# knowles-group/iterative-solver

Hardware: AMD Instinct MI355X
Metric: subspace-update GB/s (gemm_inner+axpy) at N=1e8, 8 roots; 1/2/4/8 GPU (higher is better)
Workload: dtype f64

## Files before the change

iterative-solver_amd/csrc/context.hip:

```cpp
#include <immintrin.h>

#include <unistd.h>

#include <algorithm>
#include <atomic>
#include <chrono>
#include <condition_variable>
#include <cstdio>
#include <cstdlib>
#include <cstring>
#include <memory>
#include <mutex>
#include <thread>

#include "ssp_internal.h"

namespace {
thread_local std::string g_last_error;

size_t round_block(size_t bytes) {
  if (bytes < (size_t(1) << 20)) return (bytes + 255) & ~size_t(255);
  const size_t g = size_t(2) << 20;
  return (bytes + g - 1) / g * g;
}
// ... 287 lines not shown
}

int ledger_resolve(ssp_ctx* ctx) {
  SSP_TRY_HIP(hipStreamSynchronize(ctx->stream));
  for (auto& e : ctx->ledger) {
    for (auto& pr : e.pending) {
      float ms = 0;
      SSP_TRY_HIP(hipEventElapsedTime(&ms, pr.first, pr.second));
      e.ms += ms;
      ctx->event_pool.push_back(pr.first);
      ctx->event_pool.push_back(pr.second);
    }
    e.pending.clear();
  }
  return SSP_OK;
}
}

namespace {
thread_local LedgerScope* t_scope = nullptr;
}

LedgerScope::LedgerScope(ssp_ctx* ctx, const char* op, double bytes) : ctx_(ctx) {
  if (!ctx->ledger_on) return;
  slot_ = ledger_slot(ctx, op);
  ctx->ledger[slot_].calls += 1;
  ctx->ledger[slot_].bytes += bytes;
  last_bytes_ = bytes;
  start_ = take_event(ctx);
  if (!start_) return;
  if (ctx->ledger_dispatch) {
    stop_ = take_event(ctx);
    if (!stop_) {
      ctx->event_pool.push_back(start_);
      start_ = nullptr;
      return;
    }
    prev_ = t_scope;
    t_scope = this;
    return;
  }
  (void)hipEventRecord(start_, ctx->stream);
}

bool LedgerScope::dispatch_events(hipStream_t stream, hipEvent_t* start, hipEvent_t* stop) {
  LedgerScope* s = t_scope;
  if (!s || stream != s->ctx_->stream) return false;
  *start = s->launched_ ? nullptr : s->start_;
  *stop = s->stop_;
  s->launched_ = true;
  return true;
}

void LedgerScope::detail(const std::string& tag) {
  if (slot_ < 0 || !ctx_->ledger_detail) return;
  const std::string name = ctx_->ledger[slot_].name + " [" + tag + "]";
  auto& from = ctx_->ledger[slot_];
  from.calls -= 1;
  const double b = last_bytes_;
  from.bytes -= b;
  const int to = ledger_slot(ctx_, name.c_str());
  ctx_->ledger[to].calls += 1;
  ctx_->ledger[to].bytes += b;
  slot_ = to;
}

LedgerScope::~LedgerScope() {
  if (slot_ < 0 || !start_) return;
  if (stop_) {
    t_scope = prev_;
    if (!launched_) {
      ctx_->event_pool.push_back(start_);
      ctx_->event_pool.push_back(stop_);
      return;
    }
    ctx_->ledger[slot_].pending.emplace_back(start_, stop_);
  } else {
    hipEvent_t end = take_event(ctx_);
    if (!end) return;
    (void)hipEventRecord(end, ctx_->stream);
    ctx_->ledger[slot_].pending.emplace_back(start_, end);
  }
  if (ctx_->ledger[slot_].pending.size() > 4096) (void)ledger_resolve(ctx_);
}

}

extern "C" {

int ssp_ledger_enable(ssp_ctx* ctx, int enable) {
  SSP_CHECK_CTX(ctx);
  ctx->ledger_on = enable != 0;
  return SSP_OK;
}

int ssp_ledger_reset(ssp_ctx* ctx) {
  SSP_CHECK_CTX(ctx);
  SSP_TRY(ssp::ledger_resolve(ctx));
  ctx->ledger.clear();
  return SSP_OK;
}

int ssp_ledger_reserve(ssp_ctx* ctx, int n) {
  SSP_CHECK_CTX(ctx);
  SSP_TRY(ssp::use_device(ctx));
  while (int(ctx->event_pool.size()) < n) {
    hipEvent_t e = nullptr;
    SSP_TRY_HIP(hipEventCreate(&e));
    ctx->event_pool.push_back(e);
  }
  return SSP_OK;
}

int ssp_ledger_count(ssp_ctx* ctx) {
  if (!ctx) return -1;
// ... 4 lines not shown
int ssp_ledger_entry(ssp_ctx* ctx, int i, const char** name, long long* calls, double* kernel_ms, double* bytes) {
  SSP_CHECK_CTX(ctx);
  SSP_TRY(ssp::ledger_resolve(ctx));
  if (i < 0 || size_t(i) >= ctx->ledger.size()) return ssp::set_error(SSP_ERR_ARG, "ssp_ledger_entry: bad index");
  const auto& e = ctx->ledger[i];
  if (name) *name = e.name.c_str();
  if (calls) *calls = e.calls;
  if (kernel_ms) *kernel_ms = e.ms;
  if (bytes) *bytes = e.bytes;
  return SSP_OK;
}

const char* ssp_last_error(void) { return g_last_error.c_str(); }

const char* ssp_version(void) { return "subspace_hip 0.1 (gfx950, fp64)"; }

int ssp_device_count(void) {
  int n = 0;
  if (hipGetDeviceCount(&n) != hipSuccess) return 0;
  return n;
}

int ssp_ctx_create(int device, ssp_ctx** out) {
  if (!out) return ssp::set_error(SSP_ERR_ARG, "ssp_ctx_create: null out");
  *out = nullptr;
  int ndev = 0;
  SSP_TRY_HIP(hipGetDeviceCount(&ndev));
  if (device < 0 || device >= ndev)
    return ssp::set_error(SSP_ERR_ARG, "ssp_ctx_create: device " + std::to_string(device) + " not present");
  SSP_TRY_HIP(hipSetDevice(device));
  auto* ctx = new ssp_ctx();
  ctx->device = device;
  hipDeviceProp_t prop;
  if (hipGetDeviceProperties(&prop, device) == hipSuccess && prop.multiProcessorCount > 0)
    ctx->num_cus = prop.multiProcessorCount;
  if (const char* rs = std::getenv("SSP_ROW_SHAPE")) ctx->row_stride = std::string(rs) == "stride";
  if (const char* pc = std::getenv("SSP_PUBLISH")) ctx->publish_copy = std::string(pc) == "copy";
  if (const char* ex = std::getenv("SSP_EXACT_MAX")) ctx->exact_max = size_t(std::strtoull(ex, nullptr, 10));
  if (const char* ip = std::getenv("SSP_INNER_PER_CU")) ctx->inner_per_cu = std::max(1, std::atoi(ip));
  if (const char* op = std::getenv("SSP_OUTER_WG_PER_CU")) ctx->outer_per_cu = std::max(1, std::atoi(op));
  if (const char* fp = std::getenv("SSP_FUSED_PER_CU")) ctx->fused_per_cu = std::max(1, std::atoi(fp));
  if (const char* tw = std::getenv("SSP_TRANSFORM_WIDE")) ctx->transform_wide = std::atoi(tw) != 0;
  if (const char* sm = std::getenv("SSP_SELECT_MERGE")) ctx->select_rank = std::string(sm) != "tree";
  if (const char* lt = std::getenv("SSP_LEDGER_TIMING")) ctx->ledger_dispatch = std::string(lt) == "dispatch";
  ctx->ledger_detail = std::getenv("SSP_LEDGER_DETAIL") != nullptr;
  if (const char* ss = std::getenv("SSP_SYNTH_SHAPE")) {
    ctx->synth_stride = std::string(ss) == "stride";
    ctx->synth_window = std::string(ss) == "window";
  }
  if (const char* sm = std::getenv("SSP_SYNTH_MERGE")) ctx->synth_merge = std::atoi(sm) != 0;
  if (const char* df = std::getenv("SSP_DEFER_FILL")) ctx->defer_fill = std::atoi(df) != 0;
  if (const char* dout = std::getenv("SSP_DEFER_OUTER")) ctx->outer.defer = std::atoi(dout) != 0;
  if (const char* on = std::getenv("SSP_OUTER_NORMS")) ctx->outer.norms_on = std::atoi(on) != 0;
  if (const char* ct = std::getenv("SSP_COMM_TIMEOUT_S")) {
    const double v = std::atof(ct);
    if (v > 0) ctx->comm_timeout_s = v;
  }
  if (hipStreamCreateWithFlags(&ctx->stream, hipStreamNonBlocking) != hipSuccess) {
    delete ctx;
    return ssp::set_error(SSP_ERR_HIP, "hipStreamCreate failed");
  }
  int s = ssp::ensure_partial(ctx, size_t(1) << 20);
  if (s == SSP_OK) s = ssp::ensure_result(ctx, size_t(1) << 16);
  if (s == SSP_OK) {
    const size_t bytes = sizeof(unsigned) * ssp::kFoldLine * (ssp::kFoldShards + 1);
    if (hipMalloc(reinterpret_cast<void**>(&ctx->fold_counter), bytes) != hipSuccess ||
        hipMemsetAsync(ctx->fold_counter, 0, bytes, ctx->stream) != hipSuccess)
      s = ssp::set_error(SSP_ERR_NOMEM, "allocation of the reduction counter failed");
  }
  if (s != SSP_OK) {
    ssp_ctx_destroy(ctx);
    return s;
  }
  *out = ctx;
  return SSP_OK;
}

int ssp_ctx_destroy(ssp_ctx* ctx) {
  if (!ctx) return SSP_OK;
  (void)hipSetDevice(ctx->device);
  ctx->pending_fills.clear();
  ctx->outer.pending.discard();
  (void)ssp::p2p_detach(ctx);
  if (ctx->stream) (void)hipStreamSynchronize(ctx->stream);
  if (ctx->comm) ncclCommDestroy(ctx->comm);
  if (ctx->dev_err_host) (void)hipHostFree(ctx->dev_err_host);
  for (auto& e : ctx->ledger)
    for (auto& pr : e.pending) {
      (void)hipEventDestroy(pr.first);
      (void)hipEventDestroy(pr.second);
    }
  for (auto ev : ctx->event_pool) (void)hipEventDestroy(ev);
  for (auto& b : ctx->free_blocks) (void)hipFree(b.second);
  for (auto& b : ctx->live_blocks) (void)hipFree(b.first);
  if (ctx->partial) (void)hipFree(ctx->partial);
  if (ctx->outer.norms_dev) (void)hipFree(ctx->outer.norms_dev);
  if (ctx->result_dev) (void)hipFree(ctx->result_dev);
  if (ctx->result_host) (void)hipHostFree(ctx->result_host);
  if (ctx->pub_flag) (void)hipHostFree(ctx->pub_flag);
  if (ctx->fold_counter) (void)hipFree(ctx->fold_counter);
  if (ctx->async_dev) (void)hipFree(ctx->async_dev);
  if (ctx->async_host) (void)hipHostFree(ctx->async_host);
  if (ctx->async_flag) (void)hipHostFree(ctx->async_flag);
  if (ctx->synth_mask) (void)hipFree(ctx->synth_mask);
  if (ctx->ring_dev) (void)hipFree(ctx->ring_dev);
  if (ctx->ring_host) (void)hipHostFree(ctx->ring_host);
  for (auto& r : ctx->retired_rings) {
    if (r.first) (void)hipFree(r.first);
    if (r.second) (void)hipHostFree(r.second);
  }
  if (ctx->stream) (void)hipStreamDestroy(ctx->stream);
  delete ctx;
  return SSP_OK;
}

void* ssp_ctx_stream(ssp_ctx* ctx) {
  if (!ctx) return nullptr;
  (void)ssp::enter(ctx);
  return reinterpret_cast<void*>(ctx->stream);
}

int ssp_synchronize(ssp_ctx* ctx) {
  SSP_CHECK_CTX(ctx);
  return ssp::sync_stream(ctx, "synchronize");
}

int ssp_alloc(ssp_ctx* ctx, size_t n, double** out) {
  SSP_CHECK_CTX(ctx);
  if (!out) return ssp::set_error(SSP_ERR_ARG, "ssp_alloc: null out");
  const size_t bytes = round_block(std::max<size_t>(n, 1) * sizeof(double));
  auto it = ctx->free_blocks.find(bytes);
  void* p = nullptr;
  if (it != ctx->free_blocks.end()) {
    p = it->second;
    ctx->free_blocks.erase(it);
// ... 222 lines not shown
```

iterative-solver_amd/csrc/kernels_outer.hip:

```cpp
#include <algorithm>
#include <string>
#include <vector>

#include "ssp_internal.h"

namespace {

using ssp::kBlock;
using ssp::ld2, ssp::sc1, ssp::sc2;

struct OuterArgs {
  const double* x[ssp::kOuterSrc];
  double* y[ssp::kOuterDst];
  int k;
  int m;
  int set;
  int epi_mask;
  size_t n;
  const double* alpha_dev;
  const double* scale_dev;
  double alpha[ssp::kOuterAlpha];
  double epi[ssp::kOuterDst];
  double* partial;
  ssp::FoldTail tail;
// ... 166 lines not shown
          *reinterpret_cast<double2*>(a.y[j] + 2 * p) = v;
          double s = nacc[j * U * kBlock];
          s = fma(v.x, v.x, s);
          s = fma(v.y, v.y, s);
          nacc[j * U * kBlock] = s;
        }
      }
      if ((a.n & 1) && threadIdx.x == 0) {
        const size_t e = a.n - 1;
        for (int j = 0; j < a.m; ++j) {
          double v = 0.0;
          for (int i = 0; i < a.k; ++i) v = fma(alpha(i * a.m + j), a.x[i][e], v);
          if constexpr (EPI) {
            if ((a.epi_mask >> j) & 1) v = fma(a.epi[j], a.x[a.k + j][e], v);
          }
          a.y[j][e] = v;
          nacc[j * U * kBlock] = fma(v, v, nacc[j * U * kBlock]);
        }
      }
    }
    __shared__ double red[kBlock / 64][M];
#pragma unroll
    for (int j = 0; j < M; ++j)
      if (j < a.m) {
        const double s0 = nacc[(j * U + 0) * kBlock], s1 = nacc[(j * U + 1) * kBlock];
        const double s2 = nacc[(j * U + 2) * kBlock], s3 = nacc[(j * U + 3) * kBlock];
        double v = (s0 + s1) + (s2 + s3);
#pragma unroll
        for (int off = 32; off > 0; off >>= 1) v += __shfl_down(v, off, 64);
        if (lane == 0) red[threadIdx.x >> 6][j] = v;
      }
    __syncthreads();
    if (int(threadIdx.x) < a.m) {
      double s = 0;
#pragma unroll
      for (int w = 0; w < kBlock / 64; ++w) s += red[w][threadIdx.x];
      ssp::store_partial(a.partial + size_t(blockIdx.x) * a.m + threadIdx.x, s);
    }
    ssp::fold_tail<M>(a.partial, a.tail);
    return;
  }
  if ((a.n & 1) && blockIdx.x == 0 && threadIdx.x < a.m) {
    const size_t e = a.n - 1;
    const int j = threadIdx.x;
    double v = SET ? 0.0 : sc1<SC>(a.y[j][e], scale(a.k + j));
    for (int i = 0; i < a.k; ++i) v = fma(alpha(i * a.m + j), sc1<SC>(a.x[i][e], scale(i)), v);
    if constexpr (EPI) {
      if ((a.epi_mask >> j) & 1) v = fma(a.epi[j], a.x[a.k + j][e], v);
    }
    a.y[j][e] = v;
  }
}

constexpr int kOuterNormDst = 8;
unsigned outer_norm_grid(const ssp_ctx* ctx, size_t n) { return ssp::win_grid(ctx, n, ssp::kDotU, 8); }

int outer_inst(int m) { return m <= 1 ? 1 : m <= 2 ? 2 : m <= 4 ? 4 : m <= 8 ? 8 : 16; }

template <int M, bool DEV, bool SET, bool SC, bool EPI, bool NRM>
void launch_outer_inst(ssp_ctx* ctx, unsigned grid, const OuterArgs& a) {
  SSP_LAUNCH((k_gemm_outer<M, DEV, SET, SC, EPI, NRM>), dim3(grid), dim3(kBlock), 0, ctx->stream, a);
}

template <bool DEV, bool SET, bool SC, bool EPI = false, bool NRM = false>
void launch_outer_m(ssp_ctx* ctx, unsigned grid, const OuterArgs& a) {
  switch (outer_inst(a.m)) {
    case 1: return launch_outer_inst<1, DEV, SET, SC, EPI, NRM>(ctx, grid, a);
    case 2: return launch_outer_inst<2, DEV, SET, SC, EPI, NRM>(ctx, grid, a);
    case 4: return launch_outer_inst<4, DEV, SET, SC, EPI, NRM>(ctx, grid, a);
    case 8: return launch_outer_inst<8, DEV, SET, SC, EPI, NRM>(ctx, grid, a);
    default:
      if constexpr (!NRM) launch_outer_inst<16, DEV, SET, SC, EPI, NRM>(ctx, grid, a);
  }
}

template <bool SET, bool SC, bool EPI = false, bool NRM = false>
void launch_outer_dev(ssp_ctx* ctx, unsigned grid, const OuterArgs& a) {
  a.alpha_dev ? launch_outer_m<true, SET, SC, EPI, NRM>(ctx, grid, a)
              : launch_outer_m<false, SET, SC, EPI, NRM>(ctx, grid, a);
}

int launch_outer(ssp_ctx* ctx, const OuterArgs& a) {
  const unsigned grid = a.partial ? outer_norm_grid(ctx, a.n)
                                  : ssp::stream_grid(ctx, a.n / 2 + 1, kOuterWin, unsigned(ctx->outer_per_cu));
  if (a.partial) {
    if (!a.set || a.scale_dev || a.m > kOuterNormDst || (a.epi_mask && a.k + a.m > ssp::kOuterSrc))
      return ssp::set_error(SSP_ERR_ARG, "gemm_outer: norms on a launch that cannot carry them");
    a.epi_mask ? launch_outer_dev<true, false, true, true>(ctx, grid, a)
               : launch_outer_dev<true, false, false, true>(ctx, grid, a);
  } else if (a.epi_mask) {
    if (!a.set || a.scale_dev || a.k + a.m > ssp::kOuterSrc)
      return ssp::set_error(SSP_ERR_ARG, "gemm_outer: epilogue terms on a launch that cannot carry them");
    launch_outer_dev<true, false, true>(ctx, grid, a);
  } else if (a.scale_dev) {
    a.set ? launch_outer_dev<true, true>(ctx, grid, a) : launch_outer_dev<false, true>(ctx, grid, a);
  } else {
    a.set ? launch_outer_dev<true, false>(ctx, grid, a) : launch_outer_dev<false, false>(ctx, grid, a);
  }
  SSP_TRY_HIP(hipGetLastError());
  return SSP_OK;
}

int outer_args(ssp_ctx* ctx, const double* alphas, const double* const* xx, const double* xs, int k,
               double* const* yy, const double* ys, int m, size_t n, bool set0, int i0, int j0, OuterArgs* out,
               std::string* tag) {
  OuterArgs& a = *out;
  a = OuterArgs{};
// ... 2 lines not shown
  a.set = (set0 && i0 == 0) ? 1 : 0;
  a.n = n;
  for (int i = 0; i < a.k; ++i) a.x[i] = xx[i0 + i];
  for (int j = 0; j < a.m; ++j) a.y[j] = yy[j0 + j];
  if (xs || ys) {
    std::vector<double> scl(size_t(a.k + a.m), 1.0);
    for (int i = 0; i < a.k; ++i) scl[size_t(i)] = xs ? xs[i0 + i] : 1.0;
    for (int j = 0; j < a.m; ++j) scl[size_t(a.k + j)] = (ys && i0 == 0 && !set0) ? ys[j0 + j] : 1.0;
    if (ssp::any_scaled(scl.data(), int(scl.size()))) {
      void* ps;
      SSP_TRY(ssp::upload_small(ctx, scl.data(), scl.size() * sizeof(double), &ps));
      a.scale_dev = static_cast<const double*>(ps);
    }
  }
  const bool dev = a.k * a.m > ssp::kOuterAlpha;
  std::vector<double> block(dev ? size_t(a.k) * a.m : 0);
  double* dst = dev ? block.data() : a.alpha;
  for (int i = 0; i < a.k; ++i)
    for (int j = 0; j < a.m; ++j) dst[i * a.m + j] = alphas[size_t(i0 + i) * m + j0 + j];
  if (dev) {
    void* p;
    SSP_TRY(ssp::upload_small(ctx, block.data(), block.size() * sizeof(double), &p));
    a.alpha_dev = static_cast<const double*>(p);
  }
  SSP_TRY(ssp::flush_uploads(ctx));
  *tag = ssp::shape_tag(dev ? "dev" : "arg", outer_inst(a.m), a.set, a.k, a.m, a.scale_dev != nullptr);
  return SSP_OK;
}

int launch_record(ssp_ctx* ctx, const ssp::PendingOuter::Record& r, const ssp::FoldTail* norms = nullptr) {
  const int e = r.terms();
  ssp::LedgerScope ls(ctx, r.set ? "gemm_outer_set" : "gemm_outer", 8.0 * r.n * (r.k + r.m + e));
  OuterArgs a;
  std::string tag;
  SSP_TRY(outer_args(ctx, r.alpha, r.x, nullptr, r.k, r.y, nullptr, r.m, r.n, true, 0, 0, &a, &tag));
  if (e > 0) {
    a.epi_mask = int(r.mask);
    for (int j = 0; j < r.m; ++j) {
      const bool on = (r.mask >> j) & 1u;
      a.x[r.k + j] = on ? r.ex[j] : nullptr;
      a.epi[j] = on ? r.ea[j] : 0.0;
    }
    tag += " epi" + std::to_string(e);
  }
  if (norms) {
    a.partial = ctx->partial;
    a.tail = *norms;
    tag += " nrm";
  }
  ls.detail(tag);
  return launch_outer(ctx, a);
}

int launch_outer_norms(ssp_ctx* ctx, const double* y, size_t n) {
  ssp::DeferredOuter& d = ctx->outer;
  if (!d.norms_on || !d.pending.pending()) return SSP_OK;
  const ssp::PendingOuter::Record& r = d.pending.record();
  const int m = r.m;
  if (m > kOuterNormDst || n != r.n || std::find(r.y, r.y + m, y) == r.y + m) return SSP_OK;
  d.norms.forget();
  const bool ranks = ssp::comm_attached(ctx);
  ssp::FoldTail tail{};
  int status = ssp::ensure_partial(ctx, size_t(outer_norm_grid(ctx, r.n)) * m);
  if (status == SSP_OK) status = ssp::fold_begin(ctx, m, &tail);
  if (status == SSP_OK && ranks) {
    if (!d.norms_dev && hipMalloc(reinterpret_cast<void**>(&d.norms_dev), ssp::kOuterDst * sizeof(double)) != hipSuccess)
      status = ssp::set_error(SSP_ERR_NOMEM, "hipMalloc of the norm staging failed");
    tail.out = d.norms_dev;
  }
  if (status != SSP_OK) {
    const int plain = ssp::flush_outer(ctx);
    return plain != SSP_OK ? plain : status;
  }
  d.norms.keep(r.y, m, r.n);
  d.pending.flush([&](const ssp::PendingOuter::Record& rec) { status = launch_record(ctx, rec, &tail); });
  if (status == SSP_OK && !ranks) {
    double v[ssp::kOuterDst];
    status = ssp::fold_finish(ctx, tail, v);
    if (status == SSP_OK) d.norms.set_values(v);
  }
  if (status != SSP_OK) d.norms.forget();
  return status;
}

}

namespace ssp {

int flush_outer(ssp_ctx* ctx) {
  DeferredOuter& d = ctx->outer;
  d.norms.forget();
  if (!d.pending.pending()) return SSP_OK;
  int status = SSP_OK;
  d.pending.flush([&](const PendingOuter::Record& r) { status = launch_record(ctx, r); });
  return status;
}

int outer_take_axpy(ssp_ctx* ctx, double alpha, const double* x, double xs, double* y, double ys, size_t n,
                    bool* attached) {
  DeferredOuter& d = ctx->outer;
  *attached = false;
  d.norms.forget();
  if (!d.pending.pending()) return SSP_OK;
  const bool valid = n > 0 && x && y && aligned16(x) && aligned16(y);
  if (valid && xs == 1.0 && ys == 1.0 && d.pending.attach(alpha, x, y, n)) {
    *attached = true;
    return flush_fills_over(ctx, x, n);
  }
  return flush_outer(ctx);
}

int outer_serve_dot(ssp_ctx* ctx, const double* x, double xs, const double* y, double ys, size_t n, double* out,
                    bool* served) {
  DeferredOuter& d = ctx->outer;
  *served = false;
  if (!out || x != y || xs != 1.0 || ys != 1.0) return SSP_OK;
  SSP_TRY(launch_outer_norms(ctx, y, n));
  const int j = d.norms.find(y, n);
  if (j < 0) return SSP_OK;
  *served = true;
  if (!comm_attached(ctx)) {
    *out = d.norms.value(j);
    return SSP_OK;
  }
  SSP_TRY(comm_check(ctx));
  SSP_TRY(ensure_result(ctx, 1));
  SSP_TRY_HIP(hipMemcpyAsync(ctx->result_dev, d.norms_dev + j, sizeof(double), hipMemcpyDeviceToDevice, ctx->stream));
  return reduce_fetch(ctx, out, 1);
}

}

namespace {
int gemm_outer_impl(ssp_ctx* ctx, const double* alphas, const double* const* xx, const double* xs, int k,
                    double* const* yy, const double* ys, int m, size_t n, bool set) {
  SSP_CHECK_CTX_KEEP_FILLS(ctx);
  if (m < 0 || k < 0) return ssp::set_error(SSP_ERR_ARG, "ssp_gemm_outer: negative dimension");
  if (set && k == 0) {
    for (int j = 0; j < m; ++j) SSP_TRY(ssp_fill(ctx, 0.0, yy[j], n));
    return SSP_OK;
  }
  if (m == 0 || n == 0) return SSP_OK;
  if (k == 0) {
    for (int j = 0; j < m; ++j)
      if (!set && ys && ys[j] != 1.0) SSP_TRY(ssp_scal(ctx, ys[j], yy[j], n));
    return SSP_OK;
  }
  if (!alphas) return ssp::set_error(SSP_ERR_ARG, "ssp_gemm_outer: null alphas");
  SSP_TRY(ssp::check_ptrs(xx, k, n, "ssp_gemm_outer"));
  SSP_TRY(ssp::check_ptrs(yy, m, n, "ssp_gemm_outer"));
  for (int j = 0; j < m; ++j)
    for (int i = 0; i < k; ++i)
      if (yy[j] == xx[i]) return ssp::set_error(SSP_ERR_ARG, "ssp_gemm_outer: a destination aliases a source");
  bool consume = false;
  if (!ctx->pending_fills.empty()) {
    for (int i = 0; i < k; ++i) SSP_TRY(ssp::flush_fills_over(ctx, xx[i], n));
    if (set) {
      for (int j = 0; j < m; ++j) SSP_TRY(ssp::overwrite_fills(ctx, yy[j], n));
    } else {
      consume = !ssp::any_scaled(ys, m) && !ssp::exact_mode(ctx, n);
      for (int j = 0; consume && j < m; ++j) {
        consume = ctx->pending_fills.find_exact(yy[j], n) >= 0;
        for (int i = 0; consume && i < j; ++i) consume = yy[i] != yy[j];
      }
      for (int j = 0; j < m; ++j) {
        if (consume) ctx->pending_fills.erase(ctx->pending_fills.find_exact(yy[j], n));
        else SSP_TRY(ssp::flush_fills_over(ctx, yy[j], n));
      }
    }
  }
  const bool set0 = set || consume;
  if (ctx->outer.defer && set0 && !ssp::any_scaled(xs, k) && !ssp::exact_mode(ctx, n) &&
      ctx->outer.pending.record(alphas, xx, k, yy, m, n, set))
    return SSP_OK;
  ssp::LedgerScope ls(ctx, set ? "gemm_outer_set" : "gemm_outer", 8.0 * n * (k + (set0 ? 1.0 : 2.0) * m));
  if (ssp::exact_mode(ctx, n)) return ssp::exact_outer(ctx, alphas, xx, xs, k, yy, ys, m, n, set);
  for (int j0 = 0; j0 < m; j0 += ssp::kOuterDst)
    for (int i0 = 0; i0 < k; i0 += ssp::kOuterSrc) {
      OuterArgs a;
      std::string tag;
      SSP_TRY(outer_args(ctx, alphas, xx, xs, k, yy, ys, m, n, set0, i0, j0, &a, &tag));
      if (j0 == 0 && i0 == 0) ls.detail(tag);
      SSP_TRY(launch_outer(ctx, a));
    }
  return SSP_OK;
}
}

extern "C" {

int ssp_gemm_outer(ssp_ctx* ctx, const double* alphas, const double* const* xx, int k, double* const* yy, int m,
                   size_t n) {
  return gemm_outer_impl(ctx, alphas, xx, nullptr, k, yy, nullptr, m, n, false);
}

int ssp_gemm_outer_set(ssp_ctx* ctx, const double* alphas, const double* const* xx, int k, double* const* yy, int m,
                       size_t n) {
  return gemm_outer_impl(ctx, alphas, xx, nullptr, k, yy, nullptr, m, n, true);
}

int ssp_gemm_outer_scaled(ssp_ctx* ctx, const double* alphas, const double* const* xx, const double* xs, int k,
                          double* const* yy, const double* ys, int m, size_t n) {
  return gemm_outer_impl(ctx, alphas, xx, xs, k, yy, ys, m, n, false);
}

int ssp_gemm_outer_set_scaled(ssp_ctx* ctx, const double* alphas, const double* const* xx, const double* xs, int k,
                              double* const* yy, int m, size_t n) {
  return gemm_outer_impl(ctx, alphas, xx, xs, k, yy, nullptr, m, n, true);
}

}
```

iterative-solver_amd/csrc/kernels_stream.hip:

```cpp
#include <algorithm>
#include <cmath>

#include "ssp_internal.h"

namespace {

using ssp::kBlock;
using ssp::ld2, ssp::sc1, ssp::sc2, ssp::st2;
using ssp::kWinMin;
using ssp::kWinU;
using ssp::kDotU;

__device__ __forceinline__ double block_sum(double v) {
  __shared__ double wsum[kBlock / 64];
#pragma unroll
  for (int off = 32; off > 0; off >>= 1) v += __shfl_down(v, off, 64);
  const int lane = threadIdx.x & 63, wave = threadIdx.x >> 6;
  if (lane == 0) wsum[wave] = v;
  __syncthreads();
  double s = 0;
  if (threadIdx.x == 0) {
#pragma unroll
    for (int w = 0; w < kBlock / 64; ++w) s += wsum[w];
  }
// ... 270 lines not shown
    SSP_TRY_HIP(hipGetLastError());
    return SSP_OK;
  }
  SSP_LAUNCH(k_reduce_partials, dim3(rows * cols), dim3(kBlock), 0, ctx->stream, partial, nblocks, rows, cols,
                     out, ldo, row0, col0);
  SSP_TRY_HIP(hipGetLastError());
  return SSP_OK;
}
int fill_now(ssp_ctx* ctx, double alpha, double* x, size_t n) {
  SSP_TRY(ssp::check_vec(x, n, "ssp_fill"));
  if (n == 0) return SSP_OK;
  LedgerScope ls(ctx, "fill", 8.0 * n);
  SSP_LAUNCH(k_fill, dim3(stream_grid(ctx, n / 2 + 1, 1, 64)), dim3(kBlock), 0, ctx->stream, x, n, alpha);
  SSP_TRY_HIP(hipGetLastError());
  return SSP_OK;
}

namespace {
struct FillFlusher {
  ssp_ctx* ctx;
  int status = SSP_OK;
  void operator()(double* p, size_t n) {
    const int s = fill_now(ctx, 0.0, p, n);
    if (status == SSP_OK) status = s;
  }
};
}

int flush_fills(ssp_ctx* ctx) {
  if (ctx->pending_fills.empty()) return SSP_OK;
  FillFlusher f{ctx};
  ctx->pending_fills.drain(f);
  return f.status;
}

int flush_fills_over(ssp_ctx* ctx, const void* p, size_t n) {
  if (ctx->pending_fills.empty()) return SSP_OK;
  FillFlusher f{ctx};
  ctx->pending_fills.flush_overlap(p, n, f);
  return f.status;
}

int overwrite_fills(ssp_ctx* ctx, const void* p, size_t n) {
  if (ctx->pending_fills.empty()) return SSP_OK;
  FillFlusher f{ctx};
  ctx->pending_fills.overwrite(p, n, f);
  return f.status;
}
}

extern "C" {

int ssp_fill(ssp_ctx* ctx, double alpha, double* x, size_t n) {
  SSP_CHECK_CTX_KEEP_FILLS(ctx);
  if (ctx->defer_fill && n > 0 && alpha == 0.0 && !std::signbit(alpha) && !ssp::exact_mode(ctx, n)) {
    SSP_TRY(ssp::check_vec(x, n, "ssp_fill"));
    ssp::FillFlusher f{ctx};
    ctx->pending_fills.insert(x, n, f);
    return f.status;
  }
  SSP_TRY(ssp::overwrite_fills(ctx, x, n));
  return ssp::fill_now(ctx, alpha, x, n);
}

int ssp_scal(ssp_ctx* ctx, double alpha, double* x, size_t n) {
  SSP_CHECK_CTX(ctx);
  SSP_TRY(ssp::check_vec(x, n, "ssp_scal"));
  if (n == 0) return SSP_OK;
  ssp::LedgerScope ls(ctx, "scal", 16.0 * n);
  if (n >= kWinMin)
    SSP_LAUNCH(k_scal_win, dim3(ssp::win_grid(ctx, n, kWinU, 16)), dim3(kBlock), 0, ctx->stream, x, n, alpha);
  else
    SSP_LAUNCH(k_scal, dim3(ssp::stream_grid(ctx, n / 2 + 1, 4, 64)), dim3(kBlock), 0, ctx->stream, x, n, alpha);
  SSP_TRY_HIP(hipGetLastError());
  return SSP_OK;
}

}

namespace {
int copy_impl(ssp_ctx* ctx, double alpha, double* x, const double* y, size_t n, bool scaled, const char* what) {
  SSP_CHECK_CTX_KEEP_FILLS(ctx);
  SSP_TRY(ssp::check_vec(x, n, what));
  SSP_TRY(ssp::check_vec(y, n, what));
  if (n == 0 || (x == y && !scaled)) return SSP_OK;
  if (x == y) return ssp_scal(ctx, alpha, x, n);
  SSP_TRY(ssp::flush_fills_over(ctx, y, n));
  SSP_TRY(ssp::overwrite_fills(ctx, x, n));
  ssp::LedgerScope ls(ctx, scaled ? "scal_copy" : "copy", 16.0 * n);
  if (n >= kWinMin) {
    const dim3 g(ssp::win_grid(ctx, n, kWinU, 16));
    if (scaled) SSP_LAUNCH(k_copy_win<true>, g, dim3(kBlock), 0, ctx->stream, x, y, n, alpha);
    else SSP_LAUNCH(k_copy_win<false>, g, dim3(kBlock), 0, ctx->stream, x, y, n, alpha);
  } else {
    const dim3 g(ssp::stream_grid(ctx, n / 2 + 1, 4, 64));
    if (scaled) SSP_LAUNCH(k_copy<true>, g, dim3(kBlock), 0, ctx->stream, x, y, n, alpha);
    else SSP_LAUNCH(k_copy<false>, g, dim3(kBlock), 0, ctx->stream, x, y, n, alpha);
  }
  SSP_TRY_HIP(hipGetLastError());
  return SSP_OK;
}

int axpy_impl(ssp_ctx* ctx, double alpha, const double* x, double xs, double* y, double ys, size_t n,
              const char* what) {
  SSP_CHECK_CTX_KEEP_ALL(ctx);
  bool attached = false;
  SSP_TRY(ssp::outer_take_axpy(ctx, alpha, x, xs, y, ys, n, &attached));
  if (attached) return SSP_OK;
// ... 112 lines not shown
```

iterative-solver_amd/csrc/pending_outer.h:

```cpp
#pragma once
#include <cstddef>
#include <cstdint>

namespace ssp {

class PendingOuter {
 public:
  static constexpr int kSrc = 64;
  static constexpr int kDst = 16;

  struct Record {
    double alpha[kSrc * kDst];
    const double* x[kSrc];
    double* y[kDst];
    int k = 0;
    int m = 0;
    size_t n = 0;
    bool set = false;
    double ea[kDst];
    const double* ex[kDst];
    unsigned mask = 0;

    int terms() const {
      int e = 0;
      for (int j = 0; j < m; ++j) e += (mask >> j) & 1u;
      return e;
    }
  };

  bool pending() const { return pending_; }
  const Record& record() const { return r_; }

  static bool one_launch(int k, int m) { return k >= 1 && m >= 1 && k <= kSrc && m <= kDst; }
  static bool epilogue_fits(int k, int m) { return k + m <= kSrc; }

  bool record(const double* alphas, const double* const* xx, int k, double* const* yy, int m, size_t n, bool set) {
    if (pending_ || n == 0 || !one_launch(k, m)) return false;
    for (int j = 0; j < m; ++j)
      for (int i = 0; i < j; ++i)
        if (overlap(yy[i], yy[j], n)) return false;
    for (int i = 0; i < k * m; ++i) r_.alpha[i] = alphas[i];
    for (int i = 0; i < k; ++i) r_.x[i] = xx[i];
    for (int j = 0; j < m; ++j) r_.y[j] = yy[j];
    r_.k = k;
    r_.m = m;
    r_.n = n;
    r_.set = set;
    r_.mask = 0;
    pending_ = true;
    return true;
  }

  bool attach(double alpha, const double* x, const double* y, size_t n) {
    if (!pending_ || n != r_.n || !epilogue_fits(r_.k, r_.m)) return false;
    int j = 0;
    while (j < r_.m && r_.y[j] != y) ++j;
    if (j == r_.m || ((r_.mask >> j) & 1u)) return false;
    for (int d = 0; d < r_.m; ++d)
      if (overlap(x, r_.y[d], n)) return false;
    r_.ea[j] = alpha;
    r_.ex[j] = x;
    r_.mask |= 1u << j;
    return true;
  }

  template <typename F>
  void flush(F&& launch) {
    if (!pending_) return;
    pending_ = false;
    launch(static_cast<const Record&>(r_));
  }

  void discard() { pending_ = false; }

 private:
  static bool overlap(const void* a, const void* b, size_t n) {
    const uintptr_t p = reinterpret_cast<uintptr_t>(a), q = reinterpret_cast<uintptr_t>(b);
    const size_t bytes = n * sizeof(double);
    return p < q + bytes && q < p + bytes;
  }

  Record r_;
  bool pending_ = false;
};

}
```

iterative-solver_amd/csrc/ssp_internal.h:

```cpp
#pragma once
#include <hip/hip_ext.h>
#include <hip/hip_runtime.h>
#include <rccl/rccl.h>

#include <cstddef>
#include <cstdint>
#include <map>
#include <string>
#include <unordered_map>
#include <vector>

#include "pending_fill.h"
#include "pending_outer.h"
#include "outer_norms.h"
#include "subspace_hip.h"

struct ssp_ledger_entry_t {
  std::string name;
  long long calls = 0;
  double ms = 0;
  double bytes = 0;
  std::vector<std::pair<hipEvent_t, hipEvent_t>> pending;
};

namespace ssp {
struct P2PComm;

struct DeferredOuter {
  bool defer = true;
  PendingOuter pending;
  bool norms_on = true;
  OuterNorms norms;
  double* norms_dev = nullptr;
};
}

struct ssp_ctx {
  int device = 0;
  bool ledger_on = false;
  std::vector<ssp_ledger_entry_t> ledger;
  std::vector<hipEvent_t> event_pool;
  int num_cus = 256;
  int inner_per_cu = 4;
  int outer_per_cu = 8;
  int fused_per_cu = 8;
  bool select_rank = true;
  bool transform_wide = true;
  bool synth_stride = false;
  bool ledger_dispatch = false;
  bool ledger_detail = false;
  bool synth_window = false;
  bool synth_merge = true;
  bool row_stride = false;
  bool publish_copy = false;
  bool defer_fill = true;
  ssp::PendingFills pending_fills;
  ssp::DeferredOuter outer;
  hipStream_t stream = nullptr;

  std::multimap<size_t, void*> free_blocks;
  std::unordered_map<void*, size_t> live_blocks;
  size_t bytes_in_use = 0;
  size_t bytes_cached = 0;

  double* partial = nullptr;
  size_t partial_cap = 0;
  double* result_dev = nullptr;
  double* result_host = nullptr;
  size_t result_cap = 0;
  unsigned long long* pub_flag = nullptr;
  unsigned long long pub_seq = 0;
  unsigned* fold_counter = nullptr;
  double* async_dev = nullptr;
  double* async_host = nullptr;
  unsigned long long* async_flag = nullptr;
  unsigned long long async_seq = 0;
  bool async_pending = false;
  bool async_launched = false;
  size_t async_n = 0;
  std::vector<double> async_sync;

  char* ring_host = nullptr;
  char* ring_dev = nullptr;
  size_t ring_cap = 0;
  size_t ring_head = 0;
  size_t ring_pending = 0;
  std::vector<std::pair<char*, char*>> retired_rings;

  unsigned short* synth_mask = nullptr;
  size_t synth_mask_n = 0, synth_mask_offset = 0;
  unsigned long long synth_mask_seed = 0;
  int synth_mask_rank = 0;

  ncclComm_t comm = nullptr;
  ssp_host_allreduce_fn host_allreduce = nullptr;
  ssp_host_allgather_fn host_allgather = nullptr;
  void* host_user = nullptr;
  ssp::P2PComm* p2p = nullptr;
  int nranks = 1;
  int rank = 0;
  double comm_timeout_s = 300.0;
  size_t exact_max = 2048;
  bool comm_failed = false;
  std::string comm_fail_msg;
  int* dev_err_host = nullptr;
};

namespace ssp {

constexpr int kBlock = 256;
constexpr int kInnerRows = 16;
constexpr int kInnerCols = 64;
constexpr int kOuterSrc = 64;
constexpr int kOuterDst = 16;
constexpr int kOuterAlpha = 384;
constexpr int kPrecVec = 16;
constexpr int kSelectTile = 2048;
constexpr int kWinU = 8;
constexpr size_t kWinMin = size_t(1) << 24;
constexpr int kDotU = 4;

int set_error(int code, const std::string& msg);
int hip_error(hipError_t e, const char* what);
int use_device(ssp_ctx* ctx);
int fill_now(ssp_ctx* ctx, double alpha, double* x, size_t n);
int flush_fills(ssp_ctx* ctx);
int flush_fills_over(ssp_ctx* ctx, const void* p, size_t n);
int overwrite_fills(ssp_ctx* ctx, const void* p, size_t n);
int flush_outer(ssp_ctx* ctx);
int outer_take_axpy(ssp_ctx* ctx, double alpha, const double* x, double xs, double* y, double ys, size_t n,
                    bool* attached);
int outer_serve_dot(ssp_ctx* ctx, const double* x, double xs, const double* y, double ys, size_t n, double* out,
                    bool* served);
int enter(ssp_ctx* ctx);
int ensure_partial(ssp_ctx* ctx, size_t n_doubles);
int ensure_result(ssp_ctx* ctx, size_t n_doubles);
int upload_small(ssp_ctx* ctx, const void* host, size_t bytes, void** dev);
int flush_uploads(ssp_ctx* ctx);
int allreduce_dev(ssp_ctx* ctx, double* buf, size_t n);
int agree_exact_max(ssp_ctx* ctx);
int rccl_settle(ssp_ctx* ctx, ncclResult_t r, const char* what);
int fetch_result(ssp_ctx* ctx, double* out, size_t n);
int reduce_fetch(ssp_ctx* ctx, double* out, size_t n);
int wait_flag(ssp_ctx* ctx, unsigned long long seq, bool* seen, const char* what = "reduction",
              const unsigned long long* flag = nullptr);
constexpr size_t kAsyncResults = 64 * 32;
int ensure_async(ssp_ctx* ctx);
unsigned stream_grid(const ssp_ctx* ctx, size_t work_items, unsigned per_thread, unsigned blocks_per_cu = 8);

typedef double nt_double2 __attribute__((ext_vector_type(2)));
__device__ __forceinline__ double2 ld2nt(const double* p) {
  const nt_double2 v = __builtin_nontemporal_load(reinterpret_cast<const nt_double2*>(p));
  return make_double2(v.x, v.y);
}
__device__ __forceinline__ void st2nt(double* p, double2 v) {
  const nt_double2 w = {v.x, v.y};
  __builtin_nontemporal_store(w, reinterpret_cast<nt_double2*>(p));
}
__device__ __forceinline__ double2 ld2(const double* p) { return *reinterpret_cast<const double2*>(p); }
__device__ __forceinline__ void st2(double* p, double2 v) { *reinterpret_cast<double2*>(p) = v; }
template <bool SC, bool QT = false>
__device__ __forceinline__ double sc1(double v, double s) {
  const double p = SC ? v * s : v;
  return QT ? double(float(p)) : p;
}
template <bool SC, bool QT = false>
__device__ __forceinline__ double2 sc2(double2 v, double s) {
  return make_double2(sc1<SC, QT>(v.x, s), sc1<SC, QT>(v.y, s));
}
bool aligned16(const void* p);
int check_vec(const void* p, size_t n, const char* what);
int check_ptrs(const void* const* v, int count, size_t n, const char* what);
template <typename T>
int check_ptrs(const T* const* v, int count, size_t n, const char* what) {
  return check_ptrs(reinterpret_cast<const void* const*>(v), count, n, what);
}
std::string shape_tag(const char* kind, int a, int b, int c, int d, bool sc);
bool any_scaled(const double* s, int n);

class LedgerScope {
 public:
  LedgerScope(ssp_ctx* ctx, const char* op, double bytes);
  ~LedgerScope();
  LedgerScope(const LedgerScope&) = delete;
  LedgerScope& operator=(const LedgerScope&) = delete;
  void detail(const std::string& tag);
  static bool dispatch_events(hipStream_t stream, hipEvent_t* start, hipEvent_t* stop);

 private:
  ssp_ctx* ctx_;
  int slot_ = -1;
  hipEvent_t start_ = nullptr;
  hipEvent_t stop_ = nullptr;
  bool launched_ = false;
  double last_bytes_ = 0;
  LedgerScope* prev_ = nullptr;
};

#define SSP_LAUNCH(K, G, B, SHM, ST, ...)                                                  \
  do {                                                                                    \
    hipEvent_t ssp_e0_ = nullptr, ssp_e1_ = nullptr;                                      \
    if (::ssp::LedgerScope::dispatch_events(ST, &ssp_e0_, &ssp_e1_))                      \
      hipExtLaunchKernelGGL(K, G, B, SHM, ST, ssp_e0_, ssp_e1_, 0u, __VA_ARGS__);         \
    else                                                                                  \
      hipLaunchKernelGGL(K, G, B, SHM, ST, __VA_ARGS__);                                  \
  } while (0)

template <int U, typename FW, typename F, typename FO>
__device__ __forceinline__ void for_windows_in(size_t n, unsigned bid, unsigned nb, FW&& fw, F&& f, FO&& fo) {
  const int lane = threadIdx.x & 63;
  const size_t gw = size_t(bid) * (kBlock / 64) + (threadIdx.x >> 6);
  const size_t nw = size_t(nb) * (kBlock / 64);
  const size_t n2 = n >> 1, win = 64 * size_t(U), nwin = n2 / win;
  for (size_t c = gw; c < nwin; c += nw) fw(c * win + lane);
  for (size_t i = nwin * win + size_t(bid) * kBlock + threadIdx.x; i < n2; i += size_t(nb) * kBlock) f(i);
  if ((n & 1) && bid == 0 && threadIdx.x == 0) fo(n - 1);
}
template <int U, typename FW, typename F, typename FO>
__device__ __forceinline__ void for_windows(size_t n, FW&& fw, F&& f, FO&& fo) {
  for_windows_in<U>(n, blockIdx.x, gridDim.x, static_cast<FW&&>(fw), static_cast<F&&>(f), static_cast<FO&&>(fo));
}

inline unsigned win_grid(const ssp_ctx* ctx, size_t n, int u, unsigned per_cu) {
  return stream_grid(ctx, ((n >> 1) / (64 * size_t(u)) + 1) * 64, 1, per_cu);
}

__device__ inline double block_sum256(double v) {
  __shared__ double wsum[kBlock / 64];
#pragma unroll
  for (int off = 32; off > 0; off >>= 1) v += __shfl_down(v, off, 64);
  const int lane = threadIdx.x & 63, wave = threadIdx.x >> 6;
  if (lane == 0) wsum[wave] = v;
  __syncthreads();
  double s = 0;
  if (threadIdx.x == 0) {
#pragma unroll
    for (int w = 0; w < kBlock / 64; ++w) s += wsum[w];
  }
  __syncthreads();
  return s;
}

template <int K>
__device__ inline void block_sum256_multi(double (&v)[K]) {
  __shared__ double wsum[K][kBlock / 64];
  const int lane = threadIdx.x & 63, wave = threadIdx.x >> 6;
#pragma unroll
  for (int k = 0; k < K; ++k) {
// ... 168 lines not shown
```

Baseline: 7127.

## Pair consecutive gemm_outer calls sharing alphas into one fused kernel

```diff
diff --git a/iterative-solver_amd/csrc/context.hip b/iterative-solver_amd/csrc/context.hip
--- a/iterative-solver_amd/csrc/context.hip
+++ b/iterative-solver_amd/csrc/context.hip
@@ -363,15 +363,21 @@
   return true;
 }
 
+void LedgerScope::calls(int c) {
+  if (slot_ < 0) return;
+  ctx_->ledger[slot_].calls += c - calls_;
+  calls_ = c;
+}
+
 void LedgerScope::detail(const std::string& tag) {
   if (slot_ < 0 || !ctx_->ledger_detail) return;
   const std::string name = ctx_->ledger[slot_].name + " [" + tag + "]";
   auto& from = ctx_->ledger[slot_];
-  from.calls -= 1;
+  from.calls -= calls_;
   const double b = last_bytes_;
   from.bytes -= b;
   const int to = ledger_slot(ctx_, name.c_str());
-  ctx_->ledger[to].calls += 1;
+  ctx_->ledger[to].calls += calls_;
   ctx_->ledger[to].bytes += b;
   slot_ = to;
 }
@@ -482,6 +488,7 @@
   if (const char* df = std::getenv("SSP_DEFER_FILL")) ctx->defer_fill = std::atoi(df) != 0;
   if (const char* dout = std::getenv("SSP_DEFER_OUTER")) ctx->outer.defer = std::atoi(dout) != 0;
   if (const char* on = std::getenv("SSP_OUTER_NORMS")) ctx->outer.norms_on = std::atoi(on) != 0;
+  if (const char* pr = std::getenv("SSP_OUTER_PAIR")) ctx->outer.pair_on = std::atoi(pr) != 0;
   if (const char* ct = std::getenv("SSP_COMM_TIMEOUT_S")) {
     const double v = std::atof(ct);
     if (v > 0) ctx->comm_timeout_s = v;
@@ -511,6 +518,7 @@
   (void)hipSetDevice(ctx->device);
   ctx->pending_fills.clear();
   ctx->outer.pending.discard();
+  ctx->outer.pair.discard();
   (void)ssp::p2p_detach(ctx);
   if (ctx->stream) (void)hipStreamSynchronize(ctx->stream);
   if (ctx->comm) ncclCommDestroy(ctx->comm);
diff --git a/iterative-solver_amd/csrc/kernels_outer.hip b/iterative-solver_amd/csrc/kernels_outer.hip
--- a/iterative-solver_amd/csrc/kernels_outer.hip
+++ b/iterative-solver_amd/csrc/kernels_outer.hip
@@ -242,7 +242,180 @@
   }
 }
 
+struct PairArgs {
+  const double* xp[ssp::kOuterSrc];
+  const double* xa[ssp::kOuterSrc];
+  double* yp[ssp::OuterPair::kDst];
+  double* ya[ssp::OuterPair::kDst];
+  double e[ssp::OuterPair::kDst];
+  const double* alpha_dev;
+  size_t n;
+  int k;
+  int m;
+  int mask;
+  double* partial;
+  ssp::FoldTail tail;
+};
+static_assert(sizeof(PairArgs) <= 4000, "kernel argument block too large");
+
+constexpr int kPairHalf = 2;
+template <int M, int B>
+__global__ __launch_bounds__(kBlock) void k_gemm_outer_pair(const PairArgs a) {
+  static_assert(M <= ssp::OuterPair::kDst && kOuterWin % kPairHalf == 0, "two half-windows of a dot window");
+  using ssp::ld2nt;
+  using ssp::st2nt;
+  using cdouble = const __attribute__((address_space(4))) double;
+  const auto alpha = [&](int idx) { return ((cdouble*)a.alpha_dev)[idx]; };
+  constexpr int U = kOuterWin, H = kPairHalf;
+  const int lane = threadIdx.x & 63;
+  const size_t gw = size_t(blockIdx.x) * (kBlock / 64) + (threadIdx.x >> 6);
+  const size_t nw = size_t(gridDim.x) * (kBlock / 64);
+  const size_t n2 = a.n >> 1, win = 64 * U;
+  const double2 z2 = make_double2(0, 0);
+  double* nacc = outer_norm_acc<M>() + threadIdx.x;
+#pragma unroll
+  for (int q = 0; q < M * U; ++q) nacc[q * kBlock] = 0;
+  const auto sums = [&](const double* const(&x)[ssp::kOuterSrc], size_t q0, double2(&acc)[H][M]) {
+#pragma unroll
+    for (int v = 0; v < H; ++v)
+#pragma unroll
+      for (int j = 0; j < M; ++j) acc[v][j] = z2;
+    int i = 0;
+    for (; i + B <= a.k; i += B) {
+      double2 xv[B][H];
+#pragma unroll
+      for (int b = 0; b < B; ++b)
+#pragma unroll
+        for (int v = 0; v < H; ++v) xv[b][v] = ld2nt(x[i + b] + 2 * (q0 + 64 * v));
+#pragma unroll
+      for (int b = 0; b < B; ++b)
+#pragma unroll
+        for (int j = 0; j < M; ++j) {
+          if (j < a.m) {
+            const double al = alpha((i + b) * a.m + j);
+#pragma unroll
+            for (int v = 0; v < H; ++v) {
+              acc[v][j].x = fma(al, xv[b][v].x, acc[v][j].x);
+              acc[v][j].y = fma(al, xv[b][v].y, acc[v][j].y);
+            }
+          }
+        }
+    }
+    for (; i < a.k; ++i) {
+      double2 xv[H];
+#pragma unroll
+      for (int v = 0; v < H; ++v) xv[v] = ld2nt(x[i] + 2 * (q0 + 64 * v));
+#pragma unroll
+      for (int j = 0; j < M; ++j) {
+        if (j < a.m) {
+          const double al = alpha(i * a.m + j);
+#pragma unroll
+          for (int v = 0; v < H; ++v) {
+            acc[v][j].x = fma(al, xv[v].x, acc[v][j].x);
+            acc[v][j].y = fma(al, xv[v].y, acc[v][j].y);
+          }
+        }
+      }
+    }
+  };
+  for (size_t c = gw; c < n2 / win; c += nw) {
+#pragma unroll
+    for (int h = 0; h < U / H; ++h) {
+      const size_t q0 = c * win + 64 * H * h + lane;
+      double2 ap[H][M], aa[H][M];
+      sums(a.xp, q0, ap);
+#pragma unroll
+      for (int v = 0; v < H; ++v)
+#pragma unroll
+        for (int j = 0; j < M; ++j)
+          if (j < a.m) st2nt(a.yp[j] + 2 * (q0 + 64 * v), ap[v][j]);
+      sums(a.xa, q0, aa);
+#pragma unroll
+      for (int j = 0; j < M; ++j)
+        if (j < a.m) {
+          if ((a.mask >> j) & 1) {
+            const double ea = a.e[j];
+#pragma unroll
+            for (int v = 0; v < H; ++v) {
+              aa[v][j].x = fma(ea, ap[v][j].x, aa[v][j].x);
+              aa[v][j].y = fma(ea, ap[v][j].y, aa[v][j].y);
+            }
+          }
+#pragma unroll
+          for (int v = 0; v < H; ++v) {
+            st2nt(a.ya[j] + 2 * (q0 + 64 * v), aa[v][j]);
+            double s = nacc[(j * U + H * h + v) * kBlock];
+            s = fma(aa[v][j].x, aa[v][j].x, s);
+            s = fma(aa[v][j].y, aa[v][j].y, s);
+            nacc[(j * U + H * h + v) * kBlock] = s;
+          }
+          __builtin_amdgcn_sched_barrier(0);
+        }
+    }
+  }
+  if (blockIdx.x == 0) {
+    const size_t p = (n2 / win) * win + threadIdx.x;
+    if (p < n2) {
+      for (int j = 0; j < a.m; ++j) {
+        double2 vp = z2, va = z2;
+        for (int i = 0; i < a.k; ++i) {
+          const double al = alpha(i * a.m + j);
+          const double2 xp = ld2(a.xp[i] + 2 * p), xa = ld2(a.xa[i] + 2 * p);
+          vp.x = fma(al, xp.x, vp.x);
+          vp.y = fma(al, xp.y, vp.y);
+          va.x = fma(al, xa.x, va.x);
+          va.y = fma(al, xa.y, va.y);
+        }
+        if ((a.mask >> j) & 1) {
+          va.x = fma(a.e[j], vp.x, va.x);
+          va.y = fma(a.e[j], vp.y, va.y);
+        }
+        ssp::st2(a.yp[j] + 2 * p, vp);
+        ssp::st2(a.ya[j] + 2 * p, va);
+        double s = nacc[j * U * kBlock];
+        s = fma(va.x, va.x, s);
+        s = fma(va.y, va.y, s);
+        nacc[j * U * kBlock] = s;
+      }
+    }
+    if ((a.n & 1) && threadIdx.x == 0) {
+      const size_t e = a.n - 1;
+      for (int j = 0; j < a.m; ++j) {
+        double vp = 0.0, va = 0.0;
+        for (int i = 0; i < a.k; ++i) {
+          vp = fma(alpha(i * a.m + j), a.xp[i][e], vp);
+          va = fma(alpha(i * a.m + j), a.xa[i][e], va);
+        }
+        if ((a.mask >> j) & 1) va = fma(a.e[j], vp, va);
+        a.yp[j][e] = vp;
+        a.ya[j][e] = va;
+        nacc[j * U * kBlock] = fma(va, va, nacc[j * U * kBlock]);
+      }
+    }
+  }
+  __shared__ double red[kBlock / 64][M];
+#pragma unroll
+  for (int j = 0; j < M; ++j)
+    if (j < a.m) {
+      const double s0 = nacc[(j * U + 0) * kBlock], s1 = nacc[(j * U + 1) * kBlock];
+      const double s2 = nacc[(j * U + 2) * kBlock], s3 = nacc[(j * U + 3) * kBlock];
+      double v = (s0 + s1) + (s2 + s3);
+#pragma unroll
+      for (int off = 32; off > 0; off >>= 1) v += __shfl_down(v, off, 64);
+      if (lane == 0) red[threadIdx.x >> 6][j] = v;
+    }
+  __syncthreads();
+  if (int(threadIdx.x) < a.m) {
+    double s = 0;
+#pragma unroll
+    for (int w = 0; w < kBlock / 64; ++w) s += red[w][threadIdx.x];
+    ssp::store_partial(a.partial + size_t(blockIdx.x) * a.m + threadIdx.x, s);
+  }
+  ssp::fold_tail<M>(a.partial, a.tail);
+}
+
 constexpr int kOuterNormDst = 8;
+constexpr int kPairSrc = 4;
 unsigned outer_norm_grid(const ssp_ctx* ctx, size_t n) { return ssp::win_grid(ctx, n, ssp::kDotU, 8); }
 
 int outer_inst(int m) { return m <= 1 ? 1 : m <= 2 ? 2 : m <= 4 ? 4 : m <= 8 ? 8 : 16; }
@@ -351,9 +524,62 @@
   return launch_outer(ctx, a);
 }
 
+template <int M>
+void launch_pair_inst(ssp_ctx* ctx, unsigned grid, const PairArgs& a) {
+  SSP_LAUNCH((k_gemm_outer_pair<M, kPairSrc>), dim3(grid), dim3(kBlock), 0, ctx->stream, a);
+}
+
+int launch_pair(ssp_ctx* ctx, const ssp::PendingOuter::Record& ra, const ssp::PendingOuter::Record& rb, unsigned mask,
+                const double* e, const ssp::FoldTail& norms) {
+  ssp::LedgerScope ls(ctx, rb.set ? "gemm_outer_set" : "gemm_outer", 8.0 * rb.n * (2.0 * rb.k + 2.0 * rb.m));
+  ls.calls(2);
+  PairArgs a{};
+  a.k = rb.k;
+  a.m = rb.m;
+  a.n = rb.n;
+  a.mask = int(mask);
+  for (int i = 0; i < rb.k; ++i) {
+    a.xp[i] = ra.x[i];
+    a.xa[i] = rb.x[i];
+  }
+  int terms = 0;
+  for (int j = 0; j < rb.m; ++j) {
+    a.yp[j] = ra.y[j];
+    a.ya[j] = rb.y[j];
+    const bool on = (mask >> j) & 1u;
+    a.e[j] = on ? e[j] : 0.0;
+    terms += on;
+  }
+  void* p;
+  SSP_TRY(ssp::upload_small(ctx, rb.alpha, sizeof(double) * size_t(rb.k) * size_t(rb.m), &p));
+  a.alpha_dev = static_cast<const double*>(p);
+  SSP_TRY(ssp::flush_uploads(ctx));
+  a.partial = ctx->partial;
+  a.tail = norms;
+  ls.detail(ssp::shape_tag("pair", outer_inst(rb.m), 1, rb.k, rb.m, false) + " reg" + std::to_string(terms) + " nrm");
+  const unsigned grid = outer_norm_grid(ctx, rb.n);
+  switch (outer_inst(rb.m)) {
+    case 1: launch_pair_inst<1>(ctx, grid, a); break;
+    case 2: launch_pair_inst<2>(ctx, grid, a); break;
+    case 4: launch_pair_inst<4>(ctx, grid, a); break;
+    case 8: launch_pair_inst<8>(ctx, grid, a); break;
+    default: return ssp::set_error(SSP_ERR_ARG, "gemm_outer: a pair wider than its kernel");
+  }
+  SSP_TRY_HIP(hipGetLastError());
+  return SSP_OK;
+}
+
+int unpair_outer(ssp_ctx* ctx) {
+  ssp::DeferredOuter& d = ctx->outer;
+  int status = SSP_OK;
+  d.pair.unpair(d.pending, [&](const ssp::PendingOuter::Record& r) { status = launch_record(ctx, r); });
+  return status;
+}
+
 int launch_outer_norms(ssp_ctx* ctx, const double* y, size_t n) {
   ssp::DeferredOuter& d = ctx->outer;
   if (!d.norms_on || !d.pending.pending()) return SSP_OK;
+  const bool paired = d.pair.paired();
   const ssp::PendingOuter::Record& r = d.pending.record();
   const int m = r.m;
   if (m > kOuterNormDst || n != r.n || std::find(r.y, r.y + m, y) == r.y + m) return SSP_OK;
@@ -372,7 +598,11 @@
     return plain != SSP_OK ? plain : status;
   }
   d.norms.keep(r.y, m, r.n);
-  d.pending.flush([&](const ssp::PendingOuter::Record& rec) { status = launch_record(ctx, rec, &tail); });
+  if (paired)
+    d.pair.flush(d.pending, [&](const ssp::PendingOuter::Record& ra, const ssp::PendingOuter::Record& rb, unsigned mask,
+                                const double* e) { status = launch_pair(ctx, ra, rb, mask, e, tail); });
+  else
+    d.pending.flush([&](const ssp::PendingOuter::Record& rec) { status = launch_record(ctx, rec, &tail); });
   if (status == SSP_OK && !ranks) {
     double v[ssp::kOuterDst];
     status = ssp::fold_finish(ctx, tail, v);
@@ -390,9 +620,17 @@
   DeferredOuter& d = ctx->outer;
   d.norms.forget();
   if (!d.pending.pending()) return SSP_OK;
-  int status = SSP_OK;
-  d.pending.flush([&](const PendingOuter::Record& r) { status = launch_record(ctx, r); });
+  int status = unpair_outer(ctx);
+  d.pending.flush([&](const PendingOuter::Record& r) {
+    const int s = launch_record(ctx, r);
+    if (status == SSP_OK) status = s;
+  });
   return status;
+}
+
+bool outer_keeps_fill(const ssp_ctx* ctx, const void* p, size_t n) {
+  const DeferredOuter& d = ctx->outer;
+  return d.pair_on && d.pending.pending() && p && aligned16(p) && !d.pair.touches(d.pending, p, n);
 }
 
 int outer_take_axpy(ssp_ctx* ctx, double alpha, const double* x, double xs, double* y, double ys, size_t n,
@@ -402,6 +640,13 @@
   d.norms.forget();
   if (!d.pending.pending()) return SSP_OK;
   const bool valid = n > 0 && x && y && aligned16(x) && aligned16(y);
+  if (d.pair.paired()) {
+    if (valid && xs == 1.0 && ys == 1.0 && d.pair.attach(d.pending, alpha, x, y, n)) {
+      *attached = true;
+      return SSP_OK;
+    }
+    SSP_TRY(unpair_outer(ctx));
+  }
   if (valid && xs == 1.0 && ys == 1.0 && d.pending.attach(alpha, x, y, n)) {
     *attached = true;
     return flush_fills_over(ctx, x, n);
@@ -431,9 +676,33 @@
 }
 
 namespace {
+bool pair_candidate(ssp_ctx* ctx, const double* alphas, const double* const* xx, const double* xs, int k,
+                    double* const* yy, const double* ys, int m, size_t n, bool set) {
+  ssp::DeferredOuter& d = ctx->outer;
+  if (!d.pair_on || !d.defer || !d.pending.pending()) return false;
+  if (d.pair.paired()) {
+    if (unpair_outer(ctx) != SSP_OK) return false;
+  }
+  if (!alphas || !xx || !yy || n == 0 || !ssp::PendingOuter::one_launch(k, m)) return false;
+  if (ssp::any_scaled(xs, k) || ssp::exact_mode(ctx, n)) return false;
+  for (int i = 0; i < k; ++i)
+    if (!xx[i] || !ssp::aligned16(xx[i])) return false;
+  for (int j = 0; j < m; ++j) {
+    if (!yy[j] || !ssp::aligned16(yy[j])) return false;
+    for (int i = 0; i < k; ++i)
+      if (yy[j] == xx[i]) return false;
+    if (!set && ctx->pending_fills.find_exact(yy[j], n) < 0) return false;
+  }
+  if (!set && ssp::any_scaled(ys, m)) return false;
+  return d.pair.may_pair(d.pending, alphas, xx, k, yy, m, n, set);
+}
+
 int gemm_outer_impl(ssp_ctx* ctx, const double* alphas, const double* const* xx, const double* xs, int k,
                     double* const* yy, const double* ys, int m, size_t n, bool set) {
-  SSP_CHECK_CTX_KEEP_FILLS(ctx);
+  if (!ctx) return ssp::set_error(SSP_ERR_ARG, "null ssp_ctx");
+  SSP_TRY(ssp::use_device(ctx));
+  const bool try_pair = pair_candidate(ctx, alphas, xx, xs, k, yy, ys, m, n, set);
+  if (!try_pair) SSP_TRY(ssp::flush_outer(ctx));
   if (m < 0 || k < 0) return ssp::set_error(SSP_ERR_ARG, "ssp_gemm_outer: negative dimension");
   if (set && k == 0) {
     for (int j = 0; j < m; ++j) SSP_TRY(ssp_fill(ctx, 0.0, yy[j], n));
@@ -469,6 +738,10 @@
     }
   }
   const bool set0 = set || consume;
+  if (try_pair) {
+    if (set0 && ctx->outer.pair.pair(ctx->outer.pending, alphas, xx, k, yy, m, n, set)) return SSP_OK;
+    SSP_TRY(ssp::flush_outer(ctx));
+  }
   if (ctx->outer.defer && set0 && !ssp::any_scaled(xs, k) && !ssp::exact_mode(ctx, n) &&
       ctx->outer.pending.record(alphas, xx, k, yy, m, n, set))
     return SSP_OK;
diff --git a/iterative-solver_amd/csrc/kernels_stream.hip b/iterative-solver_amd/csrc/kernels_stream.hip
--- a/iterative-solver_amd/csrc/kernels_stream.hip
+++ b/iterative-solver_amd/csrc/kernels_stream.hip
@@ -346,8 +346,10 @@
 extern "C" {
 
 int ssp_fill(ssp_ctx* ctx, double alpha, double* x, size_t n) {
-  SSP_CHECK_CTX_KEEP_FILLS(ctx);
-  if (ctx->defer_fill && n > 0 && alpha == 0.0 && !std::signbit(alpha) && !ssp::exact_mode(ctx, n)) {
+  SSP_CHECK_CTX_KEEP_ALL(ctx);
+  const bool defer = ctx->defer_fill && n > 0 && alpha == 0.0 && !std::signbit(alpha) && !ssp::exact_mode(ctx, n);
+  if (!(defer && ssp::outer_keeps_fill(ctx, x, n))) SSP_TRY(ssp::flush_outer(ctx));
+  if (defer) {
     SSP_TRY(ssp::check_vec(x, n, "ssp_fill"));
     ssp::FillFlusher f{ctx};
     ctx->pending_fills.insert(x, n, f);
diff --git a/iterative-solver_amd/csrc/pending_outer.h b/iterative-solver_amd/csrc/pending_outer.h
--- a/iterative-solver_amd/csrc/pending_outer.h
+++ b/iterative-solver_amd/csrc/pending_outer.h
@@ -1,6 +1,7 @@
 #pragma once
 #include <cstddef>
 #include <cstdint>
+#include <cstring>
 
 namespace ssp {
 
@@ -73,15 +74,118 @@
 
   void discard() { pending_ = false; }
 
- private:
+  void take(Record* out) {
+    *out = r_;
+    pending_ = false;
+  }
+
   static bool overlap(const void* a, const void* b, size_t n) {
     const uintptr_t p = reinterpret_cast<uintptr_t>(a), q = reinterpret_cast<uintptr_t>(b);
     const size_t bytes = n * sizeof(double);
     return p < q + bytes && q < p + bytes;
   }
 
+ private:
   Record r_;
   bool pending_ = false;
 };
 
+class OuterPair {
+ public:
+  using Record = PendingOuter::Record;
+  static constexpr int kDst = 8;
+
+  bool paired() const { return paired_; }
+  const Record& a() const { return a_; }
+  unsigned reg_mask() const { return mask_; }
+  double reg(int j) const { return e_[j]; }
+
+  bool may_pair(const PendingOuter& single, const double* alphas, const double* const* xx, int k, double* const* yy,
+                int m, size_t n, bool set) const {
+    if (paired_ || !single.pending() || n == 0 || !PendingOuter::one_launch(k, m)) return false;
+    const Record& a = single.record();
+    if (a.set != set || a.n != n || a.k != k || a.m != m || m > kDst || a.mask != 0) return false;
+    if (std::memcmp(a.alpha, alphas, sizeof(double) * size_t(k) * size_t(m)) != 0) return false;
+    for (int j = 0; j < m; ++j) {
+      for (int i = 0; i < j; ++i)
+        if (PendingOuter::overlap(yy[i], yy[j], n)) return false;
+      for (int i = 0; i < k; ++i)
+        if (PendingOuter::overlap(xx[i], a.y[j], n) || PendingOuter::overlap(yy[j], a.x[i], n)) return false;
+      for (int d = 0; d < m; ++d)
+        if (PendingOuter::overlap(yy[j], a.y[d], n)) return false;
+    }
+    return true;
+  }
+
+  bool pair(PendingOuter& single, const double* alphas, const double* const* xx, int k, double* const* yy, int m,
+            size_t n, bool set) {
+    if (!may_pair(single, alphas, xx, k, yy, m, n, set)) return false;
+    single.take(&a_);
+    single.record(alphas, xx, k, yy, m, n, set);
+    mask_ = 0;
+    paired_ = true;
+    return true;
+  }
+
+  bool attach(const PendingOuter& b, double alpha, const double* x, const double* y, size_t n) {
+    if (!paired_ || n != a_.n || !PendingOuter::epilogue_fits(a_.k, a_.m)) return false;
+    const Record& rb = b.record();
+    int j = 0;
+    while (j < a_.m && rb.y[j] != y) ++j;
+    if (j == a_.m || a_.y[j] != x || ((mask_ >> j) & 1u) || ((rb.mask >> j) & 1u)) return false;
+    e_[j] = alpha;
+    mask_ |= 1u << j;
+    return true;
+  }
+
+  bool touches(const PendingOuter& single, const void* p, size_t n) const {
+    return (paired_ && touches(a_, p, n)) || (single.pending() && touches(single.record(), p, n));
+  }
+
+  template <typename F>
+  void unpair(PendingOuter& b, F&& launch) {
+    if (!paired_) return;
+    paired_ = false;
+    launch(static_cast<const Record&>(a_));
+    for (int j = 0; j < a_.m; ++j)
+      if ((mask_ >> j) & 1u) b.attach(e_[j], a_.y[j], b.record().y[j], a_.n);
+    mask_ = 0;
+  }
+
+  template <typename F>
+  void flush(PendingOuter& b, F&& launch) {
+    if (!paired_) return;
+    paired_ = false;
+    Record rb;
+    b.take(&rb);
+    const unsigned mask = mask_;
+    mask_ = 0;
+    launch(static_cast<const Record&>(a_), static_cast<const Record&>(rb), mask, static_cast<const double*>(e_));
+  }
+
+  void discard() {
+    paired_ = false;
+    mask_ = 0;
+  }
+
+ private:
+  static bool touches(const Record& r, const void* p, size_t n) {
+    const uintptr_t a = reinterpret_cast<uintptr_t>(p);
+    const auto hit = [&](const void* q) {
+      const uintptr_t b = reinterpret_cast<uintptr_t>(q);
+      return a < b + r.n * sizeof(double) && b < a + n * sizeof(double);
+    };
+    for (int i = 0; i < r.k; ++i)
+      if (hit(r.x[i])) return true;
+    for (int j = 0; j < r.m; ++j)
+      if (hit(r.y[j]) || (((r.mask >> j) & 1u) && hit(r.ex[j]))) return true;
+    return false;
+  }
+
+  Record a_;
+  double e_[kDst] = {};
+  unsigned mask_ = 0;
+  bool paired_ = false;
+};
+
 }
diff --git a/iterative-solver_amd/csrc/ssp_internal.h b/iterative-solver_amd/csrc/ssp_internal.h
--- a/iterative-solver_amd/csrc/ssp_internal.h
+++ b/iterative-solver_amd/csrc/ssp_internal.h
@@ -29,6 +29,8 @@
 struct DeferredOuter {
   bool defer = true;
   PendingOuter pending;
+  bool pair_on = true;
+  OuterPair pair;
   bool norms_on = true;
   OuterNorms norms;
   double* norms_dev = nullptr;
@@ -132,6 +134,7 @@
                     bool* attached);
 int outer_serve_dot(ssp_ctx* ctx, const double* x, double xs, const double* y, double ys, size_t n, double* out,
                     bool* served);
+bool outer_keeps_fill(const ssp_ctx* ctx, const void* p, size_t n);
 int enter(ssp_ctx* ctx);
 int ensure_partial(ssp_ctx* ctx, size_t n_doubles);
 int ensure_result(ssp_ctx* ctx, size_t n_doubles);
@@ -185,6 +188,7 @@
   LedgerScope(const LedgerScope&) = delete;
   LedgerScope& operator=(const LedgerScope&) = delete;
   void detail(const std::string& tag);
+  void calls(int c);
   static bool dispatch_events(hipStream_t stream, hipEvent_t* start, hipEvent_t* stop);
 
  private:
@@ -194,6 +198,7 @@
   hipEvent_t stop_ = nullptr;
   bool launched_ = false;
   double last_bytes_ = 0;
+  int calls_ = 1;
   LedgerScope* prev_ = nullptr;
 };
 
```

Measured after the change: 7358, median of 6. 1.03x the previous value.
